# joezie/Personalized-PageRank-Algorithms-on-Neo4j

Hardware: AMD Instinct MI355X
Metric: single-source PPR queries/sec (FORA, alpha=0.15, eps=0.5) (higher is better)
Workload: dtype f64

## Files before the change

### personalized-pagerank-algorithms-on-neo4j_amd/csrc/device_io.cpp

```cpp
#include <algorithm>
#include <chrono>
#include <cstddef>
#include <cstdio>
#include <cstring>

#include "engine_internal.hpp"

using namespace pprhip;
using namespace pprhip::detail;

namespace pprhip {

std::atomic<int> g_kernel_timing{-1};
bool kernel_timing_on() {
  int v = g_kernel_timing.load(std::memory_order_relaxed);
  if (v < 0) {
    const char* e = hook_env("PPRHIP_KERNEL_TIMER");
    v = (e && e[0] == '1') ? 1 : 0;
    g_kernel_timing.store(v, std::memory_order_relaxed);
  }
  return v != 0;
}
int kernel_timing_level() {
  (void)kernel_timing_on();
// ... 90 lines not shown

int fetch_small(pprhip_graph* g, const void* dev, void* host, size_t bytes) {
  unsigned long long seq = 0;
  PPRHIP_TRY(fetch_begin(g, dev, bytes, &seq));
  return fetch_end(g, seq, dev, host, bytes);
}

int device_sum(pprhip_graph* g, const double* x, double* out, uint32_t count) {
  poll_idle(g);
  {
    SetupScope setup(g);
    PPRHIP_TRY(launch_sum(g, x, count ? count : act_n(g)));
  }
  PPRHIP_TRY(fetch_small(g, &g->ctr->sum_out, &g->h_ctr->sum_out, sizeof(double)));
  *out = g->h_ctr->sum_out;
  return PPRHIP_OK;
}

int read_dead_pops(pprhip_graph* g, pprhip_stats_t& st) {
  poll_idle(g);
  static_assert(offsetof(DevCounters, share_stored) == offsetof(DevCounters, dead_pops) + 64, "one copy for the nine");
  PPRHIP_TRY(fetch_small(g, &g->ctr->dead_pops, &g->h_ctr->dead_pops, 9 * sizeof(unsigned long long)));
  st.walk_loads = g->h_ctr->walk_loads;
  st.walk_load_lanes = g->h_ctr->walk_lanes;
  st.push_bytes += 16ull * (g->h_ctr->dead_pops - st.dead_end_pops);
  st.dead_end_pops = g->h_ctr->dead_pops;
  const uint64_t steps = g->h_ctr->walk_steps, walks = g->h_ctr->walks_total, srcs = g->h_ctr->sources_total;
  if (steps >= st.walk_steps && walks >= st.walks && srcs >= st.mc_sources) {
    const uint64_t served = std::min<uint64_t>(g->h_ctr->walks_served, walks - st.walks);
    const uint64_t shared = std::min<uint64_t>(g->h_ctr->share_served, walks - st.walks - served);
    const uint64_t more = 12ull * (steps - st.walk_steps) + 16ull * (walks - st.walks - served - shared) +
                          12ull * (served + shared) + 8ull * g->h_ctr->share_stored +
                          (served ? 24ull : 12ull) * (srcs - st.mc_sources);
#ifdef PPRHIP_TEST_HOOKS
    if (hook_env("PPRHIP_WALK_SHARE_LOG"))
      fprintf(stderr, "[walk-share] walks %llu served %llu stored %llu steps %llu\n", (unsigned long long)(walks - st.walks),
              (unsigned long long)g->h_ctr->share_served, (unsigned long long)g->h_ctr->share_stored,
              (unsigned long long)(steps - st.walk_steps));
#endif
    st.mc_bytes += more;
    ktimer().add_bytes(PPRHIP_KERNEL_WALK, more);
    st.walk_steps = steps;
    st.walks = walks;
    st.mc_sources = srcs;
  }
  return PPRHIP_OK;
}

int launch_walk_plan(pprhip_graph* g, int variant, double alpha, double rsum, long long nrw, double* target, double omega_dev,
                     const double* copy_src, double* copy_dst) {
  poll_idle(g);
  g->walk_hint = omega_dev > 0.0 ? 0ull : (unsigned long long)nrw + act_n(g);
  const double bound = omega_dev > 0.0 ? omega_dev : (double)nrw;
  if (bound + (double)g->gr->n >= (double)(1ull << kPackShift)) {
    set_error("walk budget %.0f exceeds the engine's 2^36 walk limit", bound);
    return PPRHIP_ERR_INVALID;
  }
  SetupScope setup(g);
  return launch_mc_plan(g, variant, alpha, rsum, (double)nrw, omega_dev, target, copy_src, copy_dst);
}

int launch_walk_run(pprhip_graph* g, int variant, double alpha, uint64_t seed, uint32_t stream, double* target) {
  poll_idle(g);
  ktimer().begin(PPRHIP_KERNEL_WALK, 0);
  const WalkIndex* ix = g->gr->widx;
  const WalkShare* ws = g->parent && g->parent->batch ? g->parent->batch->share : nullptr;
  if (variant == 0 && stream == 0 && ix && std::memcmp(&ix->alpha, &alpha, sizeof alpha) == 0 && ix->seed == seed) {
    PPRHIP_TRY(launch_mc_walk_indexed(g, ix, alpha, seed, target));
  } else if (variant == 0 && stream == 0 && ws && ws->on && ws->seed == seed &&
             std::memcmp(&ws->alpha, &alpha, sizeof alpha) == 0) {
    PPRHIP_CHECK_HIP(hipStreamWaitEvent(g->stream, ws->cleared, 0));
    PPRHIP_TRY(launch_mc_walk_shared(g, ws, alpha, seed, target));
  } else
    PPRHIP_TRY(launch_mc_walk(g, alpha, seed, stream, variant == 0 ? 1 : 0, target));
  ktimer().end();
  return PPRHIP_OK;
}

int run_walk_phase(pprhip_graph* g, int variant, double alpha, double rsum, long long nrw, uint64_t seed, uint32_t stream,
                   double* target, pprhip_stats_t& st, double omega_dev) {
  (void)st;
  PPRHIP_TRY(launch_walk_plan(g, variant, alpha, rsum, nrw, target, omega_dev));
  return launch_walk_run(g, variant, alpha, seed, stream, target);
}

int make_side_stream(pprhip_graph* g, hipStream_t* out, hipStream_t also) {
  *out = nullptr;
  int prio_lo = 0, prio_hi = 0;
  (void)hipDeviceGetStreamPriorityRange(&prio_lo, &prio_hi);
  HostMail* probe = nullptr;
  HostMail* probe_dev = nullptr;
  if (alloc_pinned((void**)&probe, sizeof(HostMail), hipHostMallocMapped) != PPRHIP_OK ||
      hipHostGetDevicePointer((void**)&probe_dev, probe, 0) != hipSuccess) {
    (void)hipGetLastError();
    if (probe) (void)hipHostFree(probe);
    return PPRHIP_ERR_OOM;
  }
  hipEvent_t held = nullptr, held2 = nullptr;
  if (hipEventCreateWithFlags(&held, hipEventDisableTiming) != hipSuccess ||
      hipEventCreateWithFlags(&held2, hipEventDisableTiming) != hipSuccess) {
    if (held) (void)hipEventDestroy(held);
    (void)hipHostFree(probe);
    return PPRHIP_ERR_HIP;
  }
  PPRHIP_CHECK_HIP(hipStreamSynchronize(g->stream));
// ... 52 lines not shown
```

### personalized-pagerank-algorithms-on-neo4j_amd/csrc/engine.hpp

```cpp
#pragma once

#include <atomic>
#include <cstdlib>
#include <vector>

#include "common.hpp"

namespace pprhip {

constexpr int kMaxBatch = 8;

struct DevCounters {
  unsigned long long hist[16];
  unsigned long long packed[2];
  double dead[2];
  unsigned long long dead_pops;
  unsigned long long walk_steps;
  unsigned long long walks_total;
  unsigned long long sources_total;
  unsigned long long walk_loads;
  unsigned long long walk_lanes;
  unsigned long long walks_served;
  unsigned long long share_served;
  unsigned long long share_stored;
// ... 220 lines not shown
  const double* seed_w;
  const int32_t* seed_id;
  const double* seed_e;
  unsigned int* seed_done;
  uint32_t seed_n_live, seed_n_all;
};

constexpr uint32_t kMailWords = 4112;
struct HostMail {
  unsigned long long seq;
  unsigned long long pad[7];
  unsigned long long words[kMailWords];
};

struct ClearList {
  void* p[6];
  unsigned long long bytes[6];
  int n;
};

struct TerminalTable {
  unsigned long long* off = nullptr;
  int32_t* term = nullptr;
  unsigned long long* usage = nullptr;
  std::vector<unsigned long long> h_off;
  double alpha = 0.0, density = 0.0;
  uint64_t seed = 0, total = 0;
};

struct WalkIndex : TerminalTable {};

constexpr uint32_t kWalkShareEmpty = 0xFFFFFFFFu;
constexpr int kWalkShareMinQueries = 32;
struct WalkShare : TerminalTable {
  hipEvent_t cleared = nullptr;
  bool on = false;
};

constexpr uint32_t kSweepTile = 4096;
constexpr uint32_t kSweepBestBlocks = 1024;
constexpr int kSweepHdrWords = 8;
struct SweepWs {
  unsigned long long* key[2] = {nullptr, nullptr};
  uint32_t* id[2] = {nullptr, nullptr};
  const uint32_t* order = nullptr;
  uint32_t* rank = nullptr;
  uint4* rec = nullptr;
  unsigned long long* deg = nullptr;
  unsigned long long* volx = nullptr;
  uint32_t* tile_node = nullptr;
  size_t tile_cap = 0;
  long long* delta = nullptr;
  unsigned long long* cut = nullptr;
  double* part_phi = nullptr;
  unsigned long long* part_idx = nullptr;
  unsigned long long* hdr = nullptr;
  void* tmp = nullptr;
  size_t tmp_bytes = 0;
};

constexpr uint32_t kCompactPer = 4;
constexpr uint32_t kCompactTile = 256u * kCompactPer;
struct SparseWs {
  unsigned long long* cnt = nullptr;
  unsigned long long* base = nullptr;
  size_t tile_cap = 0;
  unsigned long long* offs = nullptr;
  size_t offs_cap = 0;
  unsigned long long* val[2] = {nullptr, nullptr};
// ... 82 lines not shown
  void (*idle_hook)(void*) = nullptr;
  void* idle_arg = nullptr;
  int in_c8 = 0;
  detail::FetchPipe* fetch = nullptr;
  WalkShare* share = nullptr;
};

struct ApbsWorkspace {
  char* ws = nullptr;
  uint32_t blocks = 0, cap_t = 0, cap_f = 0;
};

}

struct pprhip_graph {
  pprhip::GraphData* gr = nullptr;
  pprhip::BatchState* batch = nullptr;
  hipStream_t stream = nullptr;
  double* acc_nz = nullptr;
  double* pn_part = nullptr;
  uint32_t* pn_ctr = nullptr;
  pprhip_graph* parent = nullptr;
  int slot_index = -1;
  pprhip::BatchSync* sync = nullptr;
  hipStream_t own_stream = nullptr;
  bool c8_via_parent = false;
  bool c8_settled = false;
  hipEvent_t c8_ev[2] = {nullptr, nullptr};
  hipEvent_t col_ev = nullptr;
  int ws_index = -1;
  bool pooled = false;
  bool has_col = false;
  uint32_t walk_waves = 0;
  bool stream_open = false;
  void* stream_obj = nullptr;
  hipEvent_t walk_ev[3] = {nullptr, nullptr, nullptr};
  pprhip::KernelTimer ktimer;
  void* in_rec = nullptr;
  pprhip::ApbsWorkspace apbs_dense, apbs_xl;
  void* apbs_board = nullptr;
  uint32_t apbs_chunk = 0;
  void* ix_stage = nullptr;
  size_t ix_stage_bytes = 0;
  uint32_t n_act = 0;
  uint32_t n_dirty = 0;
  double *residue = nullptr, *reserve = nullptr, *est = nullptr;
  double* cdense[2] = {nullptr, nullptr};
  double* cF = nullptr;
  int32_t* F[2] = {nullptr, nullptr};
  uint32_t* eoff[2] = {nullptr, nullptr};
  uint8_t* flags = nullptr;
  uint32_t* armed = nullptr;
  double sel_plan_sum = 0.0;
  uint32_t mc_phase = 0;
  uint32_t mc_last_plan = 0;
  pprhip::WalkPlanRec* mc_plan_rec2 = nullptr;
  unsigned long long walk_hint = 0;
  pprhip::WalkPlanRec* mc_plan_rec = nullptr;
  double* partial = nullptr;
  uint32_t sum_np = 0;
  uint32_t* hist = nullptr;
  unsigned long long* blk_pack = nullptr;
  double* blk_dead = nullptr;
  uint32_t* blk_ndead = nullptr;
  char* sel_blob = nullptr;
  uint32_t sel_cap = 0;
// ... 62 lines not shown
#endif
int init_kernels_dense_batch();

int launch_compact_prepared(pprhip_graph* g, int cbuf, int out_fbuf, unsigned long long* d_counter, bool backward);
int launch_count_active(pprhip_graph* g, const PushArgs& a, int seed_kind, int out_slot);
int launch_seed_list(pprhip_graph* g, const PushArgs& a, int seed_kind, int out_fbuf, unsigned long long* d_counter,
                     bool write_armed = false);
int launch_seed_dense(pprhip_graph* g, const PushArgs& a, int seed_kind, int cbuf, int out_slot, int dead_slot);
int launch_sum(pprhip_graph* g, const double* x, uint32_t n);
int launch_sum_partial(pprhip_graph* g, const double* x, uint32_t n);
bool old_small_kernels();
inline uint32_t act_n(const pprhip_graph* g) { return g->n_act ? g->n_act : g->gr->n; }
int launch_set_f64(pprhip_graph* g, double* p, uint32_t idx, double value);
int launch_permute_out(pprhip_graph* g, const double* x, double* out);
int launch_seed_init(pprhip_graph* g, int fbuf, bool topk = false);
int launch_seed_clear(pprhip_graph* g, uint32_t count);
int init_kernels_frontier();

int init_kernels_walk();
int init_kernels_select();
int init_kernels_apbs();

int launch_build_walk_rec(pprhip_graph* g);
int init_kernels_host();
int launch_publish(pprhip_graph* g, const void* src, uint32_t n_words, unsigned long long seq);
int launch_clear(pprhip_graph* g, const ClearList& L);
int launch_copy_f64(pprhip_graph* g, const double* src, double* dst, size_t n);
int launch_seed_one(pprhip_graph* g, int fbuf, int32_t node);
int launch_hold(hipStream_t stream, unsigned long long ticks);
int launch_mc_plan(pprhip_graph* g, int variant, double alpha, double rsum, double nrw, double omega_dev, double* target,
                   const double* copy_src = nullptr, double* copy_dst = nullptr);
int launch_mc_walk(pprhip_graph* g, double alpha, uint64_t seed, uint32_t stream, int no_zero_hop, double* target);
int launch_mc_walk_indexed(pprhip_graph* g, const TerminalTable* ix, double alpha, uint64_t seed, double* target);
int launch_mc_walk_shared(pprhip_graph* g, const TerminalTable* ws, double alpha, uint64_t seed, double* target);
int launch_index_build(pprhip_graph* g, const TerminalTable* ix, unsigned long long* d_steps);
int launch_survival_iter(pprhip_graph* g, const double* s_old, double* s_new, double alpha, const int32_t* d_heavy,
                         uint32_t n_heavy, unsigned long long* dmax);
uint32_t survival_heavy_degree();
int launch_pair_walk(pprhip_graph* g, const int32_t* d_src, uint32_t n_pairs, uint32_t chunks, uint64_t chunk_walks,
                     uint64_t walks, double alpha, uint64_t seed, double* d_part, unsigned long long* d_steps);
int launch_pair_reduce(pprhip_graph* g, const int32_t* d_src, const int32_t* d_pos, uint32_t n_pairs, uint32_t chunks,
                       const double* d_part, uint64_t walks, const double* survival, double* d_values);
int launch_walk_batch(pprhip_graph* g, const int32_t* d_starts, const uint64_t* d_idx, uint64_t count, double alpha,
                      uint64_t seed, uint32_t stream, int no_zero_hop, int32_t* d_term, uint32_t* d_steps);
int launch_mc_pure(pprhip_graph* g, int32_t src, uint64_t n_walks, double alpha, uint64_t seed, double inc,
                   double* target);

__host__ __device__ inline uint32_t owner_of(uint32_t v, uint32_t base, uint32_t rem) {
  const uint32_t cut = rem * (base + 1u);
  return v < cut ? v / (base + 1u) : rem + (v - cut) / base;
}

struct TripleRec {
  int32_t v, t;
  double p;
};
enum ApbsCell {
  kApNextTarget = 0,
  kApOutCount = 1,
  kApOutValid = 2,
  kApOverflowCount = 3,
  kApPops = 4,
  kApEdges = 5,
  kApListLen = 6,
  kApSmallCursor = 7,
  kApTargetsDone = 8,
  kApLevelsPosted = 9,
// ... 73 lines not shown
```

### personalized-pagerank-algorithms-on-neo4j_amd/csrc/kernels_walk.hip

```cpp
#include <algorithm>

#include "device_utils.hpp"
#include "engine.hpp"

namespace pprhip {

struct Philox {
  uint32_t x[4];
};

__device__ __forceinline__ Philox philox4x32_10(uint32_t c0, uint32_t c1, uint32_t c2, uint32_t c3, uint32_t k0,
                                                uint32_t k1) {
#pragma unroll
  for (int r = 0; r < 10; ++r) {
    const uint32_t hi0 = __umulhi(0xD2511F53u, c0), lo0 = 0xD2511F53u * c0;
    const uint32_t hi1 = __umulhi(0xCD9E8D57u, c2), lo1 = 0xCD9E8D57u * c2;
    const uint32_t n0 = hi1 ^ c1 ^ k0, n2 = hi0 ^ c3 ^ k1;
    c0 = n0; c1 = lo1; c2 = n2; c3 = lo0;
    k0 += 0x9E3779B9u;
    k1 += 0xBB67AE85u;
  }
  Philox p;
  p.x[0] = c0; p.x[1] = c1; p.x[2] = c2; p.x[3] = c3;
  return p;
// ... 205 lines not shown
constexpr uint32_t kWalkWavesPerCu = 16;

struct WalkWindow {
  unsigned long long woff[kWalkWindow + 1];
  unsigned long long ext[kWalkWindow];
  double inc[kWalkWindow];
  int32_t node[kWalkWindow];
  int32_t orig[kWalkWindow];
  uint8_t ent[kWalkWindow];
};

__device__ __forceinline__ uint32_t plan_upper_bound(const WalkPlanRec* __restrict__ plan, uint32_t n_src,
                                                     unsigned long long x, int lane) {
  uint32_t a = 0, b = n_src;
  while (a < b) {
    const uint32_t step = (b - a + 63u) / 64u;
    const unsigned long long idx = (unsigned long long)a + (unsigned long long)lane * step;
    const bool gt = idx >= b || plan[idx].woff > x;
    const unsigned long long mask = __ballot(gt);
    if (mask == 0) {
      a = (uint32_t)std::min<unsigned long long>((unsigned long long)a + 63ull * step + 1ull, b);
      continue;
    }
    const uint32_t f = (uint32_t)__builtin_ctzll(mask);
    const unsigned long long nb = (unsigned long long)a + (unsigned long long)f * step;
    if (f > 0) a = a + (f - 1u) * step + 1u;
    b = (uint32_t)std::min<unsigned long long>(nb, b);
    if (f == 0) b = a;
  }
  return a;
}

enum WalkMode : int { kWalkPlain = 0, kWalkIndexed = 1, kWalkShared = 2 };
template <int MODE>
__global__ __launch_bounds__(64) void k_mc_walk(const WalkPlanRec* __restrict__ plan_rec,
                                                 const uint4* __restrict__ walk_rec, double* __restrict__ target,
                                                 double alpha, uint32_t k0, uint32_t k1, uint32_t stream,
                                                 int no_zero_hop, DevCounters* ctr, int parity,
                                                 const unsigned long long* __restrict__ idx_off,
                                                 uint32_t* share_term, uint32_t n_nodes,
                                                 unsigned long long* __restrict__ share_usage) {
  constexpr bool INDEXED = MODE == kWalkIndexed;
  constexpr bool SHARED = MODE == kWalkShared;
  constexpr unsigned long long kNoCell = ~0ull;
  const unsigned long long plan = ctr->mc_plan[parity];
  const uint32_t n_src = (uint32_t)(plan >> kPackShift);
  const unsigned long long n_walks = plan & kPackMask;
  if (blockIdx.x == 0 && threadIdx.x == 0) {
    ctr->walks_total += n_walks;
    ctr->sources_total += n_src;
  }
  if (INDEXED && ctr->walks_over == 0ull) return;
  __shared__ WalkWindow S;
  const int lane = threadIdx.x;
  const unsigned long long groups = (n_walks + 63) / 64;
  const unsigned long long per = (groups + gridDim.x - 1) / gridDim.x * 64;
  unsigned long long cursor = (unsigned long long)blockIdx.x * per;
  if (cursor >= n_walks) return;
  const unsigned long long w_hi = cursor + per < n_walks ? cursor + per : n_walks;
  uint32_t e = plan_upper_bound(plan_rec, n_src, cursor, lane) - 1u;
  unsigned long long win_lo = cursor, win_end = cursor;
  unsigned long long steps_total = 0;
  Walker w;
  double inc = 0.0;
  bool walking = false;
  unsigned long long n_loads = 0, n_lanes = 0;
  unsigned long long cell = kNoCell;
  unsigned long long n_served = 0, n_stored = 0;
  for (;;) {
    const unsigned long long need = __ballot(!walking);
    if (need && cursor < w_hi) {
      if (cursor >= win_end) {
        win_lo = cursor;
        win_end = cursor + kWalkWindow < w_hi ? cursor + kWalkWindow : w_hi;
        __syncthreads();
        WalkPlanRec r[kWalkWindow / 64];
#pragma unroll
        for (int q = 0; q < kWalkWindow / 64; ++q) {
          const unsigned long long idx = (unsigned long long)e + (unsigned long long)(q * 64 + lane);
          if (idx < n_src) {
            r[q] = plan_rec[idx];
          } else {
            r[q].woff = n_walks;
            r[q].inc = 0.0;
            r[q].ext = 0ull;
// ... 21 lines not shown
          const int j = q * 64 + lane;
          if (j > 0 && r[q].woff >= win_lo && r[q].woff < win_end) S.ent[r[q].woff - win_lo] = (uint8_t)j;
        }
        __syncthreads();
        constexpr int kPer = kWalkWindow / 64;
        uint32_t m[kPer];
#pragma unroll
        for (int q = 0; q < kPer; ++q) {
          m[q] = S.ent[lane * kPer + q];
          if (q > 0 && m[q] < m[q - 1]) m[q] = m[q - 1];
        }
        uint32_t run = m[kPer - 1];
#pragma unroll
        for (int d = 1; d < 64; d <<= 1) {
          const uint32_t o = __shfl_up(run, d);
          if (lane >= d) run = run > o ? run : o;
        }
        uint32_t before = __shfl_up(run, 1);
        if (lane == 0) before = 0;
#pragma unroll
        for (int q = 0; q < kPer; ++q) S.ent[lane * kPer + q] = (uint8_t)(m[q] > before ? m[q] : before);
        __syncthreads();
      }
      const unsigned long long avail = win_end - cursor;
      const uint32_t rank = __popcll(need & ((1ull << lane) - 1ull));
      if (!walking && rank < avail) {
        const unsigned long long gidx = cursor + rank;
        const uint32_t j = S.ent[gidx - win_lo];
        const int32_t start = S.node[j];
        inc = S.inc[j];
        const unsigned long long sext = S.ext[j];
        const unsigned long long widx = gidx - S.woff[j];
        walker_init(w, start, sext, S.orig[j], widx, stream, no_zero_hop != 0);
        bool stored = false;
        if (INDEXED) stored = widx < idx_off[start + 1] - idx_off[start];
        if (stored) {
        } else if ((sext >> 32) == 0) {
          atomic_add_noret(&target[start], inc);
        } else if (SHARED) {
          const unsigned long long o0 = idx_off[start];
          cell = widx < idx_off[start + 1] - o0 ? o0 + widx : kNoCell;
          const uint32_t t = cell != kNoCell ? share_term[cell] : kWalkShareEmpty;
          if (t < n_nodes) {
            atomic_add_noret(&target[t], inc);
            n_served++;
          } else {
            walking = true;
          }
        } else {
          walking = true;
        }
      }
      const unsigned long long want = __popcll(need);
      cursor += want < avail ? want : avail;
      if (cursor >= win_end) {
        const uint32_t jl = S.ent[win_end - 1 - win_lo];
        e += S.woff[jl + 1] == win_end ? jl + 1u : jl;
      }
    }
    if (__ballot(walking) == 0) {
      if (cursor >= w_hi) break;
      continue;
    }
    const bool can_load = walking && w.d > 0;
    bool stopped = false;
    if (walking) {
      stopped = walker_step(w, walk_rec, alpha, k0, k1);
      if (stopped) {
        atomic_add_noret(&target[w.cur], inc);
        steps_total += w.moves;
        walking = false;
        if (SHARED && cell != kNoCell) {
          share_term[cell] = (uint32_t)w.cur;
          n_stored++;
        }
      }
    }
    const unsigned long long loaded = __ballot(can_load && !stopped);
    n_loads += loaded ? 1ull : 0ull;
    n_lanes += (unsigned long long)__popcll(loaded);
  }
  steps_total = wave_sum_u64(steps_total);
  if (lane == 0 && steps_total) atomic_add_u64(&ctr->walk_steps, steps_total);
  if (lane == 0 && n_loads) {
    atomic_add_u64(&ctr->walk_loads, n_loads);
    atomic_add_u64(&ctr->walk_lanes, n_lanes);
  }
  if (SHARED) {
    n_served = wave_sum_u64(n_served);
    n_stored = wave_sum_u64(n_stored);
    if (lane == 0 && n_served) {
      atomic_add_u64(&ctr->share_served, n_served);
      atomic_add_u64(&share_usage[0], n_served);
    }
    if (lane == 0 && n_stored) {
      atomic_add_u64(&ctr->share_stored, n_stored);
      atomic_add_u64(&share_usage[1], n_stored);
    }
  }
}

__device__ __forceinline__ uint32_t index_node_of(const unsigned long long* __restrict__ off, uint32_t a, uint32_t b,
                                                  unsigned long long p) {
  while (a < b) {
    const uint32_t mid = a + (b - a + 1u) / 2u;
    if (off[mid] <= p) a = mid;
    else b = mid - 1u;
  }
  return a;
}

__global__ __launch_bounds__(64) void k_index_build(const unsigned long long* __restrict__ off, uint32_t n,
                                                     unsigned long long total,
                                                     const unsigned long long* __restrict__ out_ext,
                                                     const uint4* __restrict__ walk_rec,
                                                     const int32_t* __restrict__ new2old, double alpha, uint32_t k0,
                                                     uint32_t k1, int32_t* __restrict__ term,
                                                     unsigned long long* __restrict__ steps_out) {
  const int lane = threadIdx.x;
  const unsigned long long groups = (total + 63) / 64;
  const unsigned long long per = (groups + gridDim.x - 1) / gridDim.x * 64;
  const unsigned long long lo = (unsigned long long)blockIdx.x * per;
  if (lo >= total) return;
  const unsigned long long hi = lo + per < total ? lo + per : total;
  const uint32_t va = index_node_of(off, 0u, n - 1u, lo);
  const uint32_t vb = index_node_of(off, va, n - 1u, hi - 1ull);
  unsigned long long cursor = lo, pos = 0, steps = 0;
  Walker w;
  bool walking = false;
  for (;;) {
    const unsigned long long need = __ballot(!walking);
// ... 357 lines not shown
  const uint64_t cap = g->sync ? 1024 : 16384;
  const uint32_t grid = (uint32_t)(b > cap ? cap : (b < 1 ? 1 : b));
  const uint32_t np = g->sum_np;
  g->sum_np = 0;
  if (variant == 1 && omega_dev > 0.0 && np > 0) {
    const uint32_t tiles = (n + 256u * kPlanItems - 1) / (256u * kPlanItems);
    hipLaunchKernelGGL(k_mc_plan_topk, dim3(std::max(1u, tiles)), dim3(256), 0, g->stream, n, g->residue, alpha, omega_dev,
                       g->partial, np, g->gr->out_ext, g->gr->new2old, plan_rec_of(g, phase), g->ctr, cell, next_cell, copy_src,
                       copy_dst);
  } else if (variant == 0)
    hipLaunchKernelGGL(k_mc_plan<0>, dim3(grid), dim3(256), 0, g->stream, n, g->residue, target, alpha, rsum, nrw,
                       omega_dev, g->gr->out_ext, g->gr->new2old, plan_rec_of(g, phase), g->ctr, cell, next_cell, copy_src, copy_dst);
  else
    hipLaunchKernelGGL(k_mc_plan<1>, dim3(grid), dim3(256), 0, g->stream, n, g->residue, target, alpha, rsum, nrw,
                       omega_dev, g->gr->out_ext, g->gr->new2old, plan_rec_of(g, phase), g->ctr, cell, next_cell, copy_src, copy_dst);
  PPRHIP_CHECK_HIP(hipGetLastError());
  return PPRHIP_OK;
}

static uint32_t mc_walk_grid(pprhip_graph* g) {
  uint32_t grid = (uint32_t)g->gr->n_cus * (g->walk_waves ? g->walk_waves
                                        : g->sync   ? kWalkWavesBeside
                                                    : kWalkWavesPerCu);
  if (g->walk_hint) grid = (uint32_t)std::min<unsigned long long>(grid, std::max<unsigned long long>((g->walk_hint + 63) / 64, 1ull));
  g->walk_hint = 0;
  return grid;
}

int launch_mc_walk(pprhip_graph* g, double alpha, uint64_t seed, uint32_t stream, int no_zero_hop, double* target) {
  const uint32_t grid = mc_walk_grid(g);
  hipLaunchKernelGGL(k_mc_walk<kWalkPlain>, dim3(grid), dim3(64), 0, g->stream, plan_rec_of(g, g->mc_last_plan),
                     reinterpret_cast<const uint4*>(g->gr->walk_rec), target, alpha, (uint32_t)seed, (uint32_t)(seed >> 32), stream,
                     no_zero_hop, g->ctr, (int)(g->mc_last_plan % 3u), (const unsigned long long*)nullptr,
                     (uint32_t*)nullptr, 0u, (unsigned long long*)nullptr);
  PPRHIP_CHECK_HIP(hipGetLastError());
  return PPRHIP_OK;
}

int launch_mc_walk_indexed(pprhip_graph* g, const TerminalTable* ix, double alpha, uint64_t seed, double* target) {
  const uint32_t grid = mc_walk_grid(g);
  const int cell = (int)(g->mc_last_plan % 3u);
  hipLaunchKernelGGL(k_index_serve, dim3(grid), dim3(64), 0, g->stream, plan_rec_of(g, g->mc_last_plan), ix->off, ix->term,
                     target, g->ctr, cell, ix->usage);
  PPRHIP_CHECK_HIP(hipGetLastError());
  hipLaunchKernelGGL(k_mc_walk<kWalkIndexed>, dim3(grid), dim3(64), 0, g->stream, plan_rec_of(g, g->mc_last_plan),
                     reinterpret_cast<const uint4*>(g->gr->walk_rec), target, alpha, (uint32_t)seed, (uint32_t)(seed >> 32), 0u,
                     1, g->ctr, cell, (const unsigned long long*)ix->off, (uint32_t*)nullptr, 0u,
                     (unsigned long long*)nullptr);
  PPRHIP_CHECK_HIP(hipGetLastError());
  return PPRHIP_OK;
}

int launch_mc_walk_shared(pprhip_graph* g, const TerminalTable* ws, double alpha, uint64_t seed, double* target) {
  const uint32_t grid = mc_walk_grid(g);
  hipLaunchKernelGGL(k_mc_walk<kWalkShared>, dim3(grid), dim3(64), 0, g->stream, plan_rec_of(g, g->mc_last_plan),
                     reinterpret_cast<const uint4*>(g->gr->walk_rec), target, alpha, (uint32_t)seed, (uint32_t)(seed >> 32), 0u,
                     1, g->ctr, (int)(g->mc_last_plan % 3u), (const unsigned long long*)ws->off, (uint32_t*)ws->term, g->gr->n,
                     ws->usage);
  PPRHIP_CHECK_HIP(hipGetLastError());
  return PPRHIP_OK;
}

int launch_index_build(pprhip_graph* g, const TerminalTable* ix, unsigned long long* d_steps) {
  if (ix->total == 0) return PPRHIP_OK;
  const uint64_t cap = (uint64_t)g->gr->n_cus * kWalkWavesPerCu;
  const uint64_t groups = (ix->total + 63) / 64;
  const uint32_t grid = (uint32_t)(groups < cap ? groups : cap);
  hipLaunchKernelGGL(k_index_build, dim3(grid), dim3(64), 0, g->stream, ix->off, g->gr->n, (unsigned long long)ix->total,
                     g->gr->out_ext, reinterpret_cast<const uint4*>(g->gr->walk_rec), g->gr->new2old, ix->alpha,
                     (uint32_t)ix->seed, (uint32_t)(ix->seed >> 32), ix->term, d_steps);
  PPRHIP_CHECK_HIP(hipGetLastError());
  return PPRHIP_OK;
}

int launch_walk_batch(pprhip_graph* g, const int32_t* d_starts, const uint64_t* d_idx, uint64_t count, double alpha,
                      uint64_t seed, uint32_t stream, int no_zero_hop, int32_t* d_term, uint32_t* d_steps) {
  if (count == 0) return PPRHIP_OK;
  uint64_t b = (count + 255) / 256;
  const uint32_t grid = (uint32_t)(b > 4096 ? 4096 : b);
  hipLaunchKernelGGL(k_walk_batch, dim3(grid), dim3(256), 0, g->stream, d_starts,
                     (const unsigned long long*)d_idx, (unsigned long long)count, g->gr->out_ext, g->gr->walk_rec, g->gr->new2old, alpha,
                     (uint32_t)seed, (uint32_t)(seed >> 32), stream, no_zero_hop, d_term, d_steps);
  PPRHIP_CHECK_HIP(hipGetLastError());
  return PPRHIP_OK;
}

int launch_mc_pure(pprhip_graph* g, int32_t src, uint64_t n_walks, double alpha, uint64_t seed, double inc,
                   double* target) {
  const uint32_t phase = g->mc_phase++;
  g->mc_last_plan = phase;
  hipLaunchKernelGGL(k_plan_single, dim3(1), dim3(1), 0, g->stream, src, inc, (unsigned long long)n_walks, g->gr->out_ext,
                     g->gr->new2old, plan_rec_of(g, phase), g->ctr, (int)(phase % 3u), (int)((phase + 1u) % 3u));
// ... 6 lines not shown
```

### personalized-pagerank-algorithms-on-neo4j_amd/csrc/walk_index.cpp

```cpp
#include <cmath>
#include <cstring>
#include <memory>
#include <new>

#include "engine_internal.hpp"

using namespace pprhip;
using namespace pprhip::detail;

namespace pprhip {
namespace detail {

int walk_offsets(const GraphData* D, double density, std::vector<unsigned long long>& h_off, uint64_t* total,
                 const char* fn) {
  try {
    h_off.resize((size_t)D->n + 1);
  } catch (const std::bad_alloc&) {
    set_error("%s: out of host memory", fn);
    return PPRHIP_ERR_OOM;
  }
  const double limit = (double)(1ull << kPackShift);
  unsigned long long run = 0;
  for (uint32_t v = 0; v < D->n; ++v) {
    h_off[v] = run;
    const uint32_t d = D->h_out_rp[v + 1] - D->h_out_rp[v];
    const double c = d ? std::ceil((double)d * density) : 0.0;
    if (!(c < limit) || (double)run + c >= limit) {
      set_error("%s: density = %g asks for 2^36 terminals or more (the engine's walk limit)", fn, density);
      return PPRHIP_ERR_INVALID;
    }
    run += (unsigned long long)c;
  }
  h_off[D->n] = run;
// ... 39 lines not shown
  PPRHIP_CHECK_HIP(hipMemcpyAsync(terminals_out, T.term + o0, sizeof(int32_t) * take, hipMemcpyDeviceToHost, g->stream));
  PPRHIP_CHECK_HIP(hipStreamSynchronize(g->stream));
  for (uint64_t i = 0; i < take; ++i)
    terminals_out[i] = (uint32_t)terminals_out[i] < g->gr->n ? g->gr->h_new2old[terminals_out[i]] : -1;
  return PPRHIP_OK;
}

static int table_usage(const TerminalTable* T, uint64_t* first, uint64_t* second, int reset) {
  unsigned long long u[2] = {0ull, 0ull};
  if (T) {
    PPRHIP_CHECK_HIP(hipDeviceSynchronize());
    PPRHIP_CHECK_HIP(hipMemcpy(u, T->usage, sizeof u, hipMemcpyDeviceToHost));
    if (reset) PPRHIP_CHECK_HIP(hipMemset(T->usage, 0, sizeof u));
  }
  if (first) *first = u[0];
  if (second) *second = u[1];
  return PPRHIP_OK;
}

static uint64_t table_bytes(const TerminalTable& T, uint32_t n, int usage_cells) {
  return 4ull * T.total + 8ull * ((uint64_t)n + 1) + 8ull * (uint64_t)usage_cells;
}

static void destroy_index(WalkIndex* ix) {
  if (ix) table_free(*ix);
  delete ix;
}

void free_walk_index(GraphData* D) {
  destroy_index(D->widx);
  D->widx = nullptr;
}

void free_walk_share(BatchState* B) {
  WalkShare* ws = B->share;
  if (!ws) return;
  table_free(*ws);
  if (ws->cleared) (void)hipEventDestroy(ws->cleared);
  delete ws;
  B->share = nullptr;
}

static int walk_share_alloc(pprhip_graph* P, double density) {
  WalkShare* ws = new (std::nothrow) WalkShare();
  if (!ws) return PPRHIP_ERR_OOM;
  P->batch->share = ws;
  PPRHIP_TRY(table_alloc(*ws, P->gr, density, 2, true, P->stream, "terminal cache"));
  PPRHIP_CHECK_HIP(hipEventCreateWithFlags(&ws->cleared, hipEventDisableTiming));
  PPRHIP_CHECK_HIP(hipStreamSynchronize(P->stream));
  return PPRHIP_OK;
}

void walk_share_begin(pprhip_graph* P, int q, double alpha, double rmax, double omega, uint64_t seed) {
  BatchState* B = P->batch;
  if (B->share) B->share->on = false;
  const char* sw = hook_env("PPRHIP_WALK_SHARE");
  if ((sw && sw[0] == '0') || q < kWalkShareMinQueries || P->gr->widx) return;
  const double density = (1.0 - alpha) * rmax * omega * (1.0 + 0x1p-20);
  if (!(density > 0.0) || !std::isfinite(density)) return;
  if (B->share && B->share->density != density) free_walk_share(B);
  if (!B->share && walk_share_alloc(P, density) != PPRHIP_OK) {
    (void)hipGetLastError();
    free_walk_share(B);
    return;
  }
  WalkShare* ws = B->share;
  if (ws->total == 0) return;
  if (hipMemsetAsync(ws->term, 0xFF, sizeof(int32_t) * (size_t)ws->total, P->stream) != hipSuccess ||
      hipEventRecord(ws->cleared, P->stream) != hipSuccess) {
    (void)hipGetLastError();
    (void)hipStreamSynchronize(P->stream);
    free_walk_share(B);
    return;
  }
  ws->alpha = alpha;
  ws->seed = seed;
  ws->on = true;
}

}
}

extern "C" {

int pprhip_walk_index_density(const pprhip_fora_conf_t* conf, double eps, double rmax, double* density_out) {
  static const char* fn = "pprhip_walk_index_density";
  PPRHIP_TRY(check_positive(eps, fn, "eps"));
  PPRHIP_TRY(check_conf(conf, fn, false));
  PPRHIP_TRY(check_threshold(rmax, fn, "rmax"));
  if (!conf || !density_out) {
    set_error("%s: null argument", fn);
    return PPRHIP_ERR_INVALID;
  }
  double rmax0 = 0.0, omega = 0.0;
  PPRHIP_TRY(pprhip_fora_whole_params(conf, eps, &rmax0, &omega));
  if (rmax == 0.0) rmax = rmax0;
  *density_out = (1.0 - conf->alpha) * rmax * omega * (1.0 + 0x1p-20);
  return PPRHIP_OK;
}

// ... 76 lines not shown
  return table_usage(g->gr->widx, served, walked, reset);
}

#ifdef PPRHIP_TEST_HOOKS
int pprhip_hook_walk_share_info(pprhip_graph_t* g, int* present, int* on, uint64_t* seed, uint64_t* cells,
                                uint64_t* bytes) {
  PPRHIP_TRY(check_graph(g, "pprhip_hook_walk_share_info"));
  const WalkShare* ws = g->batch ? g->batch->share : nullptr;
  if (present) *present = ws ? 1 : 0;
  if (on) *on = ws && ws->on ? 1 : 0;
  if (seed) *seed = ws ? ws->seed : 0;
  if (cells) *cells = ws ? ws->total : 0;
  if (bytes) *bytes = ws ? table_bytes(*ws, g->gr->n, 2) : 0;
  return PPRHIP_OK;
}

int pprhip_hook_walk_share_usage(pprhip_graph_t* g, uint64_t* served, uint64_t* stored, int reset) {
  PPRHIP_TRY(check_graph(g, "pprhip_hook_walk_share_usage"));
  return table_usage(g->batch ? g->batch->share : nullptr, served, stored, reset);
}

int pprhip_hook_walk_share_fetch(pprhip_graph_t* g, int32_t node, int32_t* terminals_out, uint64_t cap,
                                 uint64_t* count_out) {
  static const char* fn = "pprhip_hook_walk_share_fetch";
  PPRHIP_TRY(check_graph(g, fn));
  PPRHIP_TRY(check_node(g, node, fn));
  const WalkShare* ws = g->batch ? g->batch->share : nullptr;
  if (!ws || (cap && !terminals_out)) {
    set_error("%s: no terminal cache on the handle, or null output", fn);
    return PPRHIP_ERR_STATE;
  }
  return table_fetch_node(g, *ws, node, true, terminals_out, cap, count_out);
}
#endif

}
```

Before: 372.5.

## Bin shared-walk terminal deposits by node tile instead of global atomics

In the shared-terminal walk kernel, each walk's terminal node and increment are now recorded to a buffer rather than atomically added to the target vector. Four follow-up kernels then count records per node tile, build work items, scatter records into tile-sorted order, and sum each tile in LDS before writing target once per node. The aim is to replace scattered global f64 atomics with mostly coalesced writes and workgroup-local accumulation. The cost is extra device memory, four more launches, and several passes over the record buffer, which may not pay off when walk counts are modest.

```diff
diff --git a/personalized-pagerank-algorithms-on-neo4j_amd/csrc/device_io.cpp b/personalized-pagerank-algorithms-on-neo4j_amd/csrc/device_io.cpp
--- a/personalized-pagerank-algorithms-on-neo4j_amd/csrc/device_io.cpp
+++ b/personalized-pagerank-algorithms-on-neo4j_amd/csrc/device_io.cpp
@@ -146,14 +146,17 @@
     const uint64_t more = 12ull * (steps - st.walk_steps) + 16ull * (walks - st.walks - served - shared) +
                           12ull * (served + shared) + 8ull * g->h_ctr->share_stored +
                           (served ? 24ull : 12ull) * (srcs - st.mc_sources);
+    uint64_t recorded = 0;
+    if (g->walk_dep_cap && walks - st.walks >= g->walk_dep_min) recorded = std::min<uint64_t>(walks - st.walks, g->walk_dep_cap);
+    g->walk_dep_cap = g->walk_dep_min = 0;
 #ifdef PPRHIP_TEST_HOOKS
     if (hook_env("PPRHIP_WALK_SHARE_LOG"))
       fprintf(stderr, "[walk-share] walks %llu served %llu stored %llu steps %llu\n", (unsigned long long)(walks - st.walks),
               (unsigned long long)g->h_ctr->share_served, (unsigned long long)g->h_ctr->share_stored,
               (unsigned long long)(steps - st.walk_steps));
 #endif
-    st.mc_bytes += more;
-    ktimer().add_bytes(PPRHIP_KERNEL_WALK, more);
+    st.mc_bytes += more + 44ull * recorded;
+    ktimer().add_bytes(PPRHIP_KERNEL_WALK, more + 44ull * recorded);
     st.walk_steps = steps;
     st.walks = walks;
     st.mc_sources = srcs;
@@ -184,7 +187,11 @@
   } else if (variant == 0 && stream == 0 && ws && ws->on && ws->seed == seed &&
              std::memcmp(&ws->alpha, &alpha, sizeof alpha) == 0) {
     PPRHIP_CHECK_HIP(hipStreamWaitEvent(g->stream, ws->cleared, 0));
-    PPRHIP_TRY(launch_mc_walk_shared(g, ws, alpha, seed, target));
+    const hipStream_t walk_stream = g->parent->batch->walk_stream;
+    const WalkDeposit* dep = walk_stream && g->stream == walk_stream && ws->dep.on ? &ws->dep : nullptr;
+    g->walk_dep_cap = dep ? dep->a.cap : 0ull;
+    g->walk_dep_min = dep ? dep->a.min_walks : 0ull;
+    PPRHIP_TRY(launch_mc_walk_shared(g, ws, alpha, seed, target, dep));
   } else
     PPRHIP_TRY(launch_mc_walk(g, alpha, seed, stream, variant == 0 ? 1 : 0, target));
   ktimer().end();
diff --git a/personalized-pagerank-algorithms-on-neo4j_amd/csrc/engine.hpp b/personalized-pagerank-algorithms-on-neo4j_amd/csrc/engine.hpp
--- a/personalized-pagerank-algorithms-on-neo4j_amd/csrc/engine.hpp
+++ b/personalized-pagerank-algorithms-on-neo4j_amd/csrc/engine.hpp
@@ -276,9 +276,34 @@
 
 constexpr uint32_t kWalkShareEmpty = 0xFFFFFFFFu;
 constexpr int kWalkShareMinQueries = 32;
+constexpr uint32_t kDepTileShift = 11;
+constexpr uint32_t kDepMaxTiles = 4096;
+constexpr uint32_t kDepSlice = 16384;
+constexpr unsigned long long kDepMinWalks = 1ull << 18;
+struct DepositArgs {
+  uint32_t* key = nullptr;
+  double* inc = nullptr;
+  uint32_t* bkey = nullptr;
+  double* binc = nullptr;
+  uint32_t* tile_cnt = nullptr;
+  uint32_t* tile_cur = nullptr;
+  uint4* items = nullptr;
+  unsigned long long* stat = nullptr;
+  unsigned long long cap = 0, min_walks = 0;
+  uint32_t tile_shift = 0, n_tiles = 0, slice = 0, items_cap = 0, n = 0;
+};
+struct WalkDeposit {
+  DepositArgs a;
+  void* block = nullptr;
+  size_t bytes = 0;
+  unsigned long long want = 0;
+  bool on = false;
+};
+
 struct WalkShare : TerminalTable {
   hipEvent_t cleared = nullptr;
   bool on = false;
+  WalkDeposit dep;
 };
 
 constexpr uint32_t kSweepTile = 4096;
@@ -427,6 +452,7 @@
   bool pooled = false;
   bool has_col = false;
   uint32_t walk_waves = 0;
+  unsigned long long walk_dep_cap = 0, walk_dep_min = 0;
   bool stream_open = false;
   void* stream_obj = nullptr;
   hipEvent_t walk_ev[3] = {nullptr, nullptr, nullptr};
@@ -555,7 +581,8 @@
                    const double* copy_src = nullptr, double* copy_dst = nullptr);
 int launch_mc_walk(pprhip_graph* g, double alpha, uint64_t seed, uint32_t stream, int no_zero_hop, double* target);
 int launch_mc_walk_indexed(pprhip_graph* g, const TerminalTable* ix, double alpha, uint64_t seed, double* target);
-int launch_mc_walk_shared(pprhip_graph* g, const TerminalTable* ws, double alpha, uint64_t seed, double* target);
+int launch_mc_walk_shared(pprhip_graph* g, const TerminalTable* ws, double alpha, uint64_t seed, double* target,
+                          const WalkDeposit* dep);
 int launch_index_build(pprhip_graph* g, const TerminalTable* ix, unsigned long long* d_steps);
 int launch_survival_iter(pprhip_graph* g, const double* s_old, double* s_new, double alpha, const int32_t* d_heavy,
                          uint32_t n_heavy, unsigned long long* dmax);
diff --git a/personalized-pagerank-algorithms-on-neo4j_amd/csrc/kernels_walk.hip b/personalized-pagerank-algorithms-on-neo4j_amd/csrc/kernels_walk.hip
--- a/personalized-pagerank-algorithms-on-neo4j_amd/csrc/kernels_walk.hip
+++ b/personalized-pagerank-algorithms-on-neo4j_amd/csrc/kernels_walk.hip
@@ -261,6 +261,8 @@
 }
 
 enum WalkMode : int { kWalkPlain = 0, kWalkIndexed = 1, kWalkShared = 2 };
+enum WalkDepositMode : int { kDepAtomic = 0, kDepBinned = 1, kDepNone = 2 };
+constexpr uint32_t kNoSlot = 0xFFFFFFFFu;
 template <int MODE>
 __global__ __launch_bounds__(64) void k_mc_walk(const WalkPlanRec* __restrict__ plan_rec,
                                                  const uint4* __restrict__ walk_rec, double* __restrict__ target,
@@ -268,7 +270,9 @@
                                                  int no_zero_hop, DevCounters* ctr, int parity,
                                                  const unsigned long long* __restrict__ idx_off,
                                                  uint32_t* share_term, uint32_t n_nodes,
-                                                 unsigned long long* __restrict__ share_usage) {
+                                                 unsigned long long* __restrict__ share_usage, int dep_mode,
+                                                 uint32_t* __restrict__ dep_key, double* __restrict__ dep_inc,
+                                                 unsigned long long dep_cap, unsigned long long dep_min) {
   constexpr bool INDEXED = MODE == kWalkIndexed;
   constexpr bool SHARED = MODE == kWalkShared;
   constexpr unsigned long long kNoCell = ~0ull;
@@ -280,6 +284,16 @@
     ctr->sources_total += n_src;
   }
   if (INDEXED && ctr->walks_over == 0ull) return;
+  const unsigned long long rec_cap = dep_mode == kDepBinned && n_walks >= dep_min ? dep_cap : 0ull;
+  uint32_t slot = kNoSlot;
+  auto deposit = [&](uint32_t t, double x) {
+    if (slot != kNoSlot) {
+      dep_key[slot] = t;
+      dep_inc[slot] = x;
+    } else if (dep_mode != kDepNone) {
+      atomic_add_noret(&target[t], x);
+    }
+  };
   __shared__ WalkWindow S;
   const int lane = threadIdx.x;
   const unsigned long long groups = (n_walks + 63) / 64;
@@ -367,17 +381,18 @@
         const unsigned long long sext = S.ext[j];
         const unsigned long long widx = gidx - S.woff[j];
         walker_init(w, start, sext, S.orig[j], widx, stream, no_zero_hop != 0);
+        slot = gidx < rec_cap ? (uint32_t)gidx : kNoSlot;
         bool stored = false;
         if (INDEXED) stored = widx < idx_off[start + 1] - idx_off[start];
         if (stored) {
         } else if ((sext >> 32) == 0) {
-          atomic_add_noret(&target[start], inc);
+          deposit((uint32_t)start, inc);
         } else if (SHARED) {
           const unsigned long long o0 = idx_off[start];
           cell = widx < idx_off[start + 1] - o0 ? o0 + widx : kNoCell;
           const uint32_t t = cell != kNoCell ? share_term[cell] : kWalkShareEmpty;
           if (t < n_nodes) {
-            atomic_add_noret(&target[t], inc);
+            deposit(t, inc);
             n_served++;
           } else {
             walking = true;
@@ -402,7 +417,7 @@
     if (walking) {
       stopped = walker_step(w, walk_rec, alpha, k0, k1);
       if (stopped) {
-        atomic_add_noret(&target[w.cur], inc);
+        deposit((uint32_t)w.cur, inc);
         steps_total += w.moves;
         walking = false;
         if (SHARED && cell != kNoCell) {
@@ -432,6 +447,138 @@
       atomic_add_u64(&ctr->share_stored, n_stored);
       atomic_add_u64(&share_usage[1], n_stored);
     }
+  }
+}
+
+__device__ __forceinline__ unsigned long long dep_records(const DepositArgs& a, const DevCounters* ctr, int parity) {
+  const unsigned long long n_walks = ctr->mc_plan[parity] & kPackMask;
+  if (n_walks < a.min_walks) return 0ull;
+  return n_walks < a.cap ? n_walks : a.cap;
+}
+
+__device__ __forceinline__ void dep_share(unsigned long long n_rec, uint32_t* lo, uint32_t* hi) {
+  const unsigned long long per = ((n_rec + gridDim.x - 1) / gridDim.x + 255ull) / 256ull * 256ull;
+  const unsigned long long a = (unsigned long long)blockIdx.x * per, b = a + per;
+  *lo = (uint32_t)(a < n_rec ? a : n_rec);
+  *hi = (uint32_t)(b < n_rec ? b : n_rec);
+}
+
+__device__ __forceinline__ uint32_t dep_tile_of(const DepositArgs& a, uint32_t key) {
+  const uint32_t t = key >> a.tile_shift;
+  return t < a.n_tiles ? t : a.n_tiles - 1u;
+}
+
+__device__ __forceinline__ void dep_count_share(const DepositArgs& a, uint32_t lo, uint32_t hi, uint32_t* hist) {
+  for (uint32_t t = threadIdx.x; t < a.n_tiles; t += 256u) hist[t] = 0u;
+  __syncthreads();
+  for (uint32_t i = lo + threadIdx.x; i < hi; i += 256u) atomicAdd(&hist[dep_tile_of(a, a.key[i])], 1u);
+  __syncthreads();
+}
+
+__global__ __launch_bounds__(256) void k_dep_count(DepositArgs a, const DevCounters* ctr, int parity) {
+  const unsigned long long n_rec = dep_records(a, ctr, parity);
+  if (n_rec == 0) return;
+  __shared__ uint32_t hist[kDepMaxTiles];
+  uint32_t lo, hi;
+  dep_share(n_rec, &lo, &hi);
+  if (lo >= hi) return;
+  dep_count_share(a, lo, hi, hist);
+  for (uint32_t t = threadIdx.x; t < a.n_tiles; t += 256u) {
+    const uint32_t c = hist[t];
+    if (c) atomicAdd(&a.tile_cnt[t], c);
+  }
+}
+
+__global__ __launch_bounds__(256) void k_dep_items(DepositArgs a, const DevCounters* ctr, int parity) {
+  const unsigned long long n_rec = dep_records(a, ctr, parity);
+  if (n_rec == 0) return;
+  __shared__ uint32_t s_scan[4];
+  const uint32_t per = (a.n_tiles + 255u) / 256u;
+  const uint32_t t_lo = threadIdx.x * per < a.n_tiles ? threadIdx.x * per : a.n_tiles;
+  const uint32_t t_hi = t_lo + per < a.n_tiles ? t_lo + per : a.n_tiles;
+  uint32_t recs = 0, its = 0;
+  for (uint32_t t = t_lo; t < t_hi; ++t) {
+    const uint32_t c = a.tile_cnt[t];
+    recs += c;
+    its += (c + a.slice - 1u) / a.slice;
+  }
+  uint32_t recs_all, its_all;
+  uint32_t base = block_excl_scan_256<uint32_t>(recs, s_scan, &recs_all);
+  uint32_t ib = block_excl_scan_256<uint32_t>(its, s_scan, &its_all);
+  for (uint32_t t = t_lo; t < t_hi; ++t) {
+    const uint32_t c = a.tile_cnt[t];
+    a.tile_cur[t] = base;
+    a.tile_cnt[t] = 0u;
+    const uint32_t k_n = (c + a.slice - 1u) / a.slice;
+    for (uint32_t k = 0; k < k_n; ++k) {
+      const uint32_t first = k * a.slice;
+      const uint32_t len = c - first < a.slice ? c - first : a.slice;
+      if (ib + k < a.items_cap) a.items[ib + k] = make_uint4(t, base + first, len, k_n > 1u ? 1u : 0u);
+    }
+    base += c;
+    ib += k_n;
+  }
+  if (threadIdx.x == 0) {
+    const unsigned long long n_walks = ctr->mc_plan[parity] & kPackMask;
+    a.stat[0] = its_all < a.items_cap ? its_all : a.items_cap;
+    a.stat[1] += 1ull;
+    a.stat[2] += n_rec;
+    a.stat[3] += n_walks - n_rec;
+  }
+}
+
+__global__ __launch_bounds__(256) void k_dep_scatter(DepositArgs a, const DevCounters* ctr, int parity) {
+  const unsigned long long n_rec = dep_records(a, ctr, parity);
+  if (n_rec == 0) return;
+  __shared__ uint32_t hist[kDepMaxTiles];
+  uint32_t lo, hi;
+  dep_share(n_rec, &lo, &hi);
+  if (lo >= hi) return;
+  dep_count_share(a, lo, hi, hist);
+  for (uint32_t t = threadIdx.x; t < a.n_tiles; t += 256u) {
+    const uint32_t c = hist[t];
+    hist[t] = c ? atomicAdd(&a.tile_cur[t], c) : 0u;
+  }
+  __syncthreads();
+  for (uint32_t i = lo + threadIdx.x; i < hi; i += 256u) {
+    const uint32_t key = a.key[i];
+    const double x = a.inc[i];
+    const uint32_t pos = atomicAdd(&hist[dep_tile_of(a, key)], 1u);
+    if (pos < n_rec) {
+      a.bkey[pos] = key;
+      a.binc[pos] = x;
+    }
+  }
+}
+
+__global__ __launch_bounds__(256) void k_dep_sum(DepositArgs a, const DevCounters* ctr, int parity,
+                                                  double* __restrict__ target) {
+  const unsigned long long n_rec = dep_records(a, ctr, parity);
+  if (n_rec == 0) return;
+  __shared__ double acc[1u << kDepTileShift];
+  const uint32_t n_items = (uint32_t)a.stat[0];
+  const uint32_t width = 1u << a.tile_shift;
+  for (uint32_t it = blockIdx.x; it < n_items; it += gridDim.x) {
+    const uint4 item = a.items[it];
+    const uint32_t v0 = item.x << a.tile_shift;
+    for (uint32_t j = threadIdx.x; j < width; j += 256u) acc[j] = 0.0;
+    __syncthreads();
+    for (uint32_t i = threadIdx.x; i < item.z; i += 256u) {
+      const unsigned long long p = (unsigned long long)item.y + i;
+      if (p >= n_rec) break;
+      const uint32_t off = a.bkey[p] - v0;
+      if (off < width) (void)__hip_atomic_fetch_add(&acc[off], a.binc[p], __ATOMIC_RELAXED, __HIP_MEMORY_SCOPE_WORKGROUP);
+    }
+    __syncthreads();
+    for (uint32_t j = threadIdx.x; j < width; j += 256u) {
+      const double x = acc[j];
+      const uint32_t v = v0 + j;
+      if (x != 0.0 && v < a.n) {
+        if (item.w) atomic_add_noret(&target[v], x);
+        else target[v] = target[v] + x;
+      }
+    }
+    __syncthreads();
   }
 }
 
@@ -855,7 +1002,8 @@
   hipLaunchKernelGGL(k_mc_walk<kWalkPlain>, dim3(grid), dim3(64), 0, g->stream, plan_rec_of(g, g->mc_last_plan),
                      reinterpret_cast<const uint4*>(g->gr->walk_rec), target, alpha, (uint32_t)seed, (uint32_t)(seed >> 32), stream,
                      no_zero_hop, g->ctr, (int)(g->mc_last_plan % 3u), (const unsigned long long*)nullptr,
-                     (uint32_t*)nullptr, 0u, (unsigned long long*)nullptr);
+                     (uint32_t*)nullptr, 0u, (unsigned long long*)nullptr, (int)kDepAtomic, (uint32_t*)nullptr,
+                     (double*)nullptr, 0ull, 0ull);
   PPRHIP_CHECK_HIP(hipGetLastError());
   return PPRHIP_OK;
 }
@@ -869,18 +1017,32 @@
   hipLaunchKernelGGL(k_mc_walk<kWalkIndexed>, dim3(grid), dim3(64), 0, g->stream, plan_rec_of(g, g->mc_last_plan),
                      reinterpret_cast<const uint4*>(g->gr->walk_rec), target, alpha, (uint32_t)seed, (uint32_t)(seed >> 32), 0u,
                      1, g->ctr, cell, (const unsigned long long*)ix->off, (uint32_t*)nullptr, 0u,
-                     (unsigned long long*)nullptr);
+                     (unsigned long long*)nullptr, (int)kDepAtomic, (uint32_t*)nullptr, (double*)nullptr, 0ull, 0ull);
   PPRHIP_CHECK_HIP(hipGetLastError());
   return PPRHIP_OK;
 }
 
-int launch_mc_walk_shared(pprhip_graph* g, const TerminalTable* ws, double alpha, uint64_t seed, double* target) {
+int launch_mc_walk_shared(pprhip_graph* g, const TerminalTable* ws, double alpha, uint64_t seed, double* target,
+                          const WalkDeposit* dep) {
   const uint32_t grid = mc_walk_grid(g);
+  const char* sw = hook_env("PPRHIP_WALK_DEPOSIT");
+  const int dep_mode = sw && sw[0] == 'n' ? kDepNone : dep && dep->on ? kDepBinned : kDepAtomic;
+  const DepositArgs none;
+  const DepositArgs& a = dep_mode == kDepBinned ? dep->a : none;
+  const int cell = (int)(g->mc_last_plan % 3u);
   hipLaunchKernelGGL(k_mc_walk<kWalkShared>, dim3(grid), dim3(64), 0, g->stream, plan_rec_of(g, g->mc_last_plan),
                      reinterpret_cast<const uint4*>(g->gr->walk_rec), target, alpha, (uint32_t)seed, (uint32_t)(seed >> 32), 0u,
-                     1, g->ctr, (int)(g->mc_last_plan % 3u), (const unsigned long long*)ws->off, (uint32_t*)ws->term, g->gr->n,
-                     ws->usage);
-  PPRHIP_CHECK_HIP(hipGetLastError());
+                     1, g->ctr, cell, (const unsigned long long*)ws->off, (uint32_t*)ws->term, g->gr->n, ws->usage, dep_mode,
+                     a.key, a.inc, (unsigned long long)a.cap, (unsigned long long)a.min_walks);
+  PPRHIP_CHECK_HIP(hipGetLastError());
+  if (dep_mode == kDepBinned) {
+    const uint32_t wg = (uint32_t)g->gr->n_cus;
+    hipLaunchKernelGGL(k_dep_count, dim3(wg), dim3(256), 0, g->stream, a, (const DevCounters*)g->ctr, cell);
+    hipLaunchKernelGGL(k_dep_items, dim3(1), dim3(256), 0, g->stream, a, (const DevCounters*)g->ctr, cell);
+    hipLaunchKernelGGL(k_dep_scatter, dim3(wg), dim3(256), 0, g->stream, a, (const DevCounters*)g->ctr, cell);
+    hipLaunchKernelGGL(k_dep_sum, dim3(wg), dim3(256), 0, g->stream, a, (const DevCounters*)g->ctr, cell, target);
+    PPRHIP_CHECK_HIP(hipGetLastError());
+  }
   return PPRHIP_OK;
 }
 
diff --git a/personalized-pagerank-algorithms-on-neo4j_amd/csrc/walk_index.cpp b/personalized-pagerank-algorithms-on-neo4j_amd/csrc/walk_index.cpp
--- a/personalized-pagerank-algorithms-on-neo4j_amd/csrc/walk_index.cpp
+++ b/personalized-pagerank-algorithms-on-neo4j_amd/csrc/walk_index.cpp
@@ -1,4 +1,6 @@
+#include <algorithm>
 #include <cmath>
+#include <cstdlib>
 #include <cstring>
 #include <memory>
 #include <new>
@@ -104,9 +106,15 @@
   D->widx = nullptr;
 }
 
+static void free_walk_deposit(WalkDeposit& d) {
+  if (d.block) (void)hipFree(d.block);
+  d = WalkDeposit();
+}
+
 void free_walk_share(BatchState* B) {
   WalkShare* ws = B->share;
   if (!ws) return;
+  free_walk_deposit(ws->dep);
   table_free(*ws);
   if (ws->cleared) (void)hipEventDestroy(ws->cleared);
   delete ws;
@@ -121,6 +129,77 @@
   PPRHIP_CHECK_HIP(hipEventCreateWithFlags(&ws->cleared, hipEventDisableTiming));
   PPRHIP_CHECK_HIP(hipStreamSynchronize(P->stream));
   return PPRHIP_OK;
+}
+
+static unsigned long long hook_number(const char* name, unsigned long long dflt) {
+  const char* e = hook_env(name);
+  return e && e[0] ? std::strtoull(e, nullptr, 10) : dflt;
+}
+
+static void walk_deposit_begin(pprhip_graph* P, WalkShare* ws) {
+  WalkDeposit& d = ws->dep;
+  d.on = false;
+  const char* sw = hook_env("PPRHIP_WALK_DEPOSIT");
+  if (sw && sw[0] == 'a') return;
+  const uint32_t n = P->gr->n;
+  uint32_t shift = 0;
+  for (unsigned long long t = hook_number("PPRHIP_WALK_DEPOSIT_TILE", 1ull << kDepTileShift); t > 1; t >>= 1) shift++;
+  if (shift < 4 || shift > kDepTileShift) shift = kDepTileShift;
+  const unsigned long long slice = std::min<unsigned long long>(
+      std::max<unsigned long long>(hook_number("PPRHIP_WALK_DEPOSIT_SLICE", kDepSlice), 16ull), kDepSlice);
+  unsigned long long cap = std::min<unsigned long long>(ws->total + n, (1ull << 31) - 1ull);
+  cap = std::min(cap, std::max<unsigned long long>(hook_number("PPRHIP_WALK_DEPOSIT_CAP", cap), 1ull));
+  const unsigned long long n_tiles = ((unsigned long long)n + (1ull << shift) - 1ull) >> shift;
+  if (n_tiles == 0 || n_tiles > kDepMaxTiles) return;
+  if (d.block && (d.want != cap || d.a.tile_shift != shift || d.a.slice != slice)) free_walk_deposit(d);
+  if (!d.block) {
+    auto up = [](size_t b) { return (b + 255) / 256 * 256; };
+    const size_t fixed = up(4 * n_tiles) * 2 + up(16 * (n_tiles + cap / slice + 1)) + up(4 * sizeof(unsigned long long));
+    size_t free_b = 0, total_b = 0;
+    if (hipMemGetInfo(&free_b, &total_b) != hipSuccess) {
+      (void)hipGetLastError();
+      return;
+    }
+    unsigned long long fit = cap;
+    if (fixed + 2 * (up(4 * fit) + up(8 * fit)) > free_b / 4) {
+      if (free_b / 4 < fixed + 4096) return;
+      fit = (free_b / 4 - fixed - 4096) / 24;
+    }
+    if (fit == 0) return;
+    const size_t bytes = fixed + 2 * (up(4 * fit) + up(8 * fit));
+    char* b = nullptr;
+    if (alloc_dev((void**)&b, bytes) != PPRHIP_OK) {
+      (void)hipGetLastError();
+      return;
+    }
+    d.block = b;
+    d.bytes = bytes;
+    d.want = cap;
+    DepositArgs& a = d.a;
+    a.cap = fit;
+    a.tile_shift = shift;
+    a.n_tiles = (uint32_t)n_tiles;
+    a.slice = (uint32_t)slice;
+    a.items_cap = (uint32_t)(n_tiles + cap / slice + 1);
+    a.n = n;
+    a.key = (uint32_t*)b;    b += up(4 * fit);
+    a.bkey = (uint32_t*)b;   b += up(4 * fit);
+    a.inc = (double*)b;      b += up(8 * fit);
+    a.binc = (double*)b;     b += up(8 * fit);
+    a.tile_cnt = (uint32_t*)b;  b += up(4 * n_tiles);
+    a.tile_cur = (uint32_t*)b;  b += up(4 * n_tiles);
+    a.items = (uint4*)b;     b += up(16 * (size_t)a.items_cap);
+    a.stat = (unsigned long long*)b;
+    if (hipMemsetAsync(a.tile_cnt, 0, up(4 * n_tiles), P->stream) != hipSuccess ||
+        hipMemsetAsync(a.stat, 0, 4 * sizeof(unsigned long long), P->stream) != hipSuccess) {
+      (void)hipGetLastError();
+      (void)hipStreamSynchronize(P->stream);
+      free_walk_deposit(d);
+      return;
+    }
+  }
+  d.a.min_walks = hook_number("PPRHIP_WALK_DEPOSIT_MIN", kDepMinWalks);
+  d.on = true;
 }
 
 void walk_share_begin(pprhip_graph* P, int q, double alpha, double rmax, double omega, uint64_t seed) {
@@ -138,6 +217,7 @@
   }
   WalkShare* ws = B->share;
   if (ws->total == 0) return;
+  walk_deposit_begin(P, ws);
   if (hipMemsetAsync(ws->term, 0xFF, sizeof(int32_t) * (size_t)ws->total, P->stream) != hipSuccess ||
       hipEventRecord(ws->cleared, P->stream) != hipSuccess) {
     (void)hipGetLastError();
@@ -280,6 +360,35 @@
   }
   return table_fetch_node(g, *ws, node, true, terminals_out, cap, count_out);
 }
+
+int pprhip_hook_walk_deposit_info(pprhip_graph_t* g, int* present, int* on, uint64_t* cap, uint32_t* tile,
+                                  uint32_t* n_tiles, uint32_t* slice, uint64_t* bytes) {
+  PPRHIP_TRY(check_graph(g, "pprhip_hook_walk_deposit_info"));
+  const WalkShare* ws = g->batch ? g->batch->share : nullptr;
+  const WalkDeposit* d = ws && ws->dep.block ? &ws->dep : nullptr;
+  if (present) *present = d ? 1 : 0;
+  if (on) *on = d && d->on ? 1 : 0;
+  if (cap) *cap = d ? d->a.cap : 0;
+  if (tile) *tile = d ? 1u << d->a.tile_shift : 0;
+  if (n_tiles) *n_tiles = d ? d->a.n_tiles : 0;
+  if (slice) *slice = d ? d->a.slice : 0;
+  if (bytes) *bytes = d ? d->bytes : 0;
+  return PPRHIP_OK;
+}
+
+int pprhip_hook_walk_deposit_usage(pprhip_graph_t* g, uint64_t* stat_out, int reset) {
+  PPRHIP_TRY(check_graph(g, "pprhip_hook_walk_deposit_usage"));
+  const WalkShare* ws = g->batch ? g->batch->share : nullptr;
+  unsigned long long u[4] = {0ull, 0ull, 0ull, 0ull};
+  if (ws && ws->dep.block) {
+    PPRHIP_CHECK_HIP(hipDeviceSynchronize());
+    PPRHIP_CHECK_HIP(hipMemcpy(u, ws->dep.a.stat, sizeof u, hipMemcpyDeviceToHost));
+    if (reset) PPRHIP_CHECK_HIP(hipMemset(ws->dep.a.stat, 0, sizeof u));
+  }
+  if (stat_out)
+    for (int i = 0; i < 4; ++i) stat_out[i] = u[i];
+  return PPRHIP_OK;
+}
 #endif
 
 }
```

New measurement: 409.0 (median of 6 runs). 1.1x the previous value.
